# flydog-sdr/FlyDog_SDR_GPS

Hardware: AMD Instinct MI355X
Metric: IQ Msamples/s ingested (waterfall + GPS acq); value = GPS acq, BASELINE configs[1] (higher is better)
Workload: dtype f32

## Files before the change

### flydog_sdr_gps_amd/csrc/kg_acq.hip

```cpp
#include "kg_common.h"
#include "kg_fft.h"
#include "kg_acq_tables.h"

#include <math.h>
#include <stdlib.h>
#include <vector>

#define SUB      4096
#define NTAPS    31
#define DECIM    4


enum { SRC_BITS = 0, SRC_IQ16 = 1, SRC_CHIPS = 2 };

__constant__ float c_hb_even[16] = {
    -0.010233f,  0.010668f, -0.016324f,  0.024377f, -0.036482f,  0.056990f, -0.101993f,
     0.316926f,  0.316926f, -0.101993f,  0.056990f, -0.036482f,  0.024377f, -0.016324f,
     0.010668f, -0.010233f,
};
#define HB_CENTRE 0.500009f

KG_DEV float bipolar(int bit) { return bit ? -1.0f : 1.0f; }

template <int SRC>
KG_DEV cf acq_source(const void *__restrict__ src, int i, int nvalid, int nchips, int boc)
{
    if (i >= nvalid) return cf{0.f, 0.f};
    if constexpr (SRC == SRC_BITS) {
        const uint8_t *p = (const uint8_t *) src;
        const int bit = (p[i >> 3] >> (i & 7)) & 1;
        const int ph = i & 3;
        const int ls = ph < 2, lc = (ph == 0) | (ph == 3);
        return cf{bipolar(bit ^ ls), bipolar(bit ^ lc)};
    } else if constexpr (SRC == SRC_IQ16) {
        const short2 v = ((const short2 *) src)[i];
        const float a = (float) v.x, b = (float) v.y;
        switch (i & 3) {
        case 0:  return cf{a, b};
        case 1:  return cf{b, -a};
        case 2:  return cf{-a, -b};
        default: return cf{-b, a};
        }
    } else {
        const uint8_t *p = (const uint8_t *) src;
        const int chip = p[(i >> 4) % nchips];
        const int b11 = boc ? ((i & 15) >= 8) : 0;
        return cf{bipolar(chip ^ b11), 0.f};
    }
}

KG_DEV cf hb_tap(const float2 *x)
{
    cf acc = kg_scale(kg_ld(&x[0]), c_hb_even[0]);
#pragma unroll
    for (int j = 1; j < 16; j++) acc = acc + kg_scale(kg_ld(&x[2 * j]), c_hb_even[j]);
    acc = acc + kg_scale(kg_ld(&x[(NTAPS - 1) / 2]), HB_CENTRE);
    return acc;
}

#define FE_TILE 256
#define FE_NY1  (2 * FE_TILE + NTAPS - 2)
#define FE_NX   (2 * FE_NY1 + NTAPS - 2)

template <int SRC>
__global__ __launch_bounds__(256) void acq_frontend_kernel(const uint8_t *__restrict__ src,
                                                          size_t src_stride, int nvalid, int nchips, int boc,
                                                          float2 *__restrict__ td, int fft_len)
{
    __shared__ float2 xs[FE_NX + 1];
    __shared__ float2 y1[FE_NY1 + 1];
    const int tid = threadIdx.x;
    const int o0 = blockIdx.x * FE_TILE;
    const void *s = src + (size_t) blockIdx.y * src_stride;
    for (int u = tid; u < FE_NX; u += 256) kg_st(&xs[u], acq_source<SRC>(s, 4 * o0 + u, nvalid, nchips, boc));
    __syncthreads();
    for (int u = tid; u < FE_NY1; u += 256) kg_st(&y1[u], hb_tap(&xs[2 * u]));
    __syncthreads();
    kg_st(&td[(size_t) blockIdx.y * fft_len + o0 + tid], hb_tap(&y1[2 * tid]));
}

#define STAMP(i)                                                                      \
    do {                                                                              \
        if (STAMPS) {                                                                 \
            __builtin_amdgcn_sched_barrier(0);                                        \
            if (threadIdx.x == 0 && blockIdx.x == 0 && blockIdx.y == 0)               \
                stamps[i] = __builtin_amdgcn_s_memrealtime();                         \
            __builtin_amdgcn_sched_barrier(0);                                        \
        }                                                                             \
    } while (0)

template <bool STAMPS>
__global__ __launch_bounds__(256) void acq_fft_sub_kernel(const float2 *__restrict__ td,
                                                         float2 *__restrict__ scratch,
                                                         const float2 *__restrict__ tab4096, int P,
                                                         unsigned long long *__restrict__ stamps)
{
    extern __shared__ __attribute__((aligned(16))) float2 smem[];
    const int t = threadIdx.x, g = blockIdx.x;
    const float2 *in = td + (size_t) blockIdx.y * P * SUB;
    float2 *out = scratch + ((size_t) blockIdx.y * P + g) * SUB;
    STAMP(0);
    cf x[16], y[16];
#pragma unroll
    for (int j = 0; j < 16; j++) x[j] = kg_ld(&in[P * (t + 256 * j) + g]);
    kg_tw4096 tw;
    kg_tw4096_load(tw, tab4096, t);
    if (STAMPS) { asm volatile("s_waitcnt vmcnt(0)" ::: "memory"); }
    STAMP(1);
    kg_subfft4096<-1>(x, y, smem, smem + SUB, tw, t);
    STAMP(2);
#pragma unroll
    for (int m = 0; m < 16; m++) kg_st(&out[t + 256 * m], y[m]);
    if (STAMPS) { asm volatile("s_waitcnt vmcnt(0)" ::: "memory"); }
    STAMP(3);
}

template <int P>
__global__ __launch_bounds__(256) void acq_fft_combine_kernel(const float2 *__restrict__ scratch,
                                                             float2 *__restrict__ planes,
                                                             float2 *__restrict__ planes_b,
                                                             size_t planes_stride,
                                                             const float2 *__restrict__ tabN,
                                                             int halo)
{
    static_assert(P == 4 || P == 16, "N = 16384 or 65536");
    const int k = blockIdx.x * 256 + threadIdx.x;
    const float2 *f = scratch + (size_t) blockIdx.y * (P * SUB);
    cf v[P];
    v[0] = kg_ld(&f[k]);
#pragma unroll
    for (int g = 1; g < P; g++) v[g] = kg_cmulc(kg_ld(&f[g * SUB + k]), kg_ld(&tabN[g * k]));
    cf fq[P];
    if constexpr (P == 4) {
        kg_radix4<-1>(v[0], v[1], v[2], v[3]);
#pragma unroll
        for (int q = 0; q < 4; q++) fq[q] = v[q];
    } else {
        kg_radix16<-1>(v, fq);
    }
    if (planes) {
        const int row = 2 * (256 + 2 * halo), plane = 8 * row;
        float2 *o = planes + (size_t) blockIdx.y * planes_stride + (size_t) (k & (P - 1)) * plane;
#pragma unroll
        for (int q = 0; q < P; q++) {
            const int k1 = k / P + (SUB / P) * q;
            const int tt = k1 & 255, j = k1 >> 8;
            kg_st(&o[(j >> 1) * row + 2 * (tt + halo) + (j & 1)], fq[q]);
            if (tt < halo) {
                const int jj = (j - 1) & 15;
                kg_st(&o[(jj >> 1) * row + 2 * (tt + 256 + halo) + (jj & 1)], fq[q]);
            }
            if (tt >= 256 - halo) {
                const int jj = (j + 1) & 15;
                kg_st(&o[(jj >> 1) * row + 2 * (tt - 256 + halo) + (jj & 1)], fq[q]);
            }
        }
    }
    if (planes_b) {
        const int row = 2 * (512 + 2 * halo), plane = 4 * row;
        float2 *o = planes_b + (size_t) blockIdx.y * planes_stride + (size_t) (k & (P - 1)) * plane;
#pragma unroll
        for (int q = 0; q < P; q++) {
            const int k1 = k / P + (SUB / P) * q;
            const int ii = k1 & 511, j = k1 >> 9;
            kg_st(&o[(j >> 1) * row + 2 * (ii + halo) + (j & 1)], fq[q]);
            if (ii < halo) {
                const int jj = (j - 1) & 7;
                kg_st(&o[(jj >> 1) * row + 2 * (ii + 512 + halo) + (jj & 1)], fq[q]);
            }
            if (ii >= 512 - halo) {
                const int jj = (j + 1) & 7;
                kg_st(&o[(jj >> 1) * row + 2 * (ii - 512 + halo) + (jj & 1)], fq[q]);
            }
        }
    }
}

struct acq_red { float p; int i; float s; int pad; };

#define ACQ_CLAIM_STRIDE 32
#define ACQ_LDS_BYTES (2 * SUB * sizeof(float2) + 16)

struct __attribute__((aligned(16))) acq_part { float p; int i; float s; int pad; };

struct acq_pair_desc {
    int data_off;
    int code_off;
    int limit;
    int out;
};

struct acq_cell_desc { int data_off, code_off, dop, limit, out; };

struct acq_walk {
    int npairs;
    int ndop, dop_lo;
};

template <int P, bool STAMPS = false>
__global__ __launch_bounds__(256, 2) void acq_correlate_kernel(
    const float2 *__restrict__ data,
    const float2 *__restrict__ code,
    const float2 *__restrict__ tab4096, const float2 *__restrict__ tabN,
    const float2 *__restrict__ comb,
    const acq_pair_desc *__restrict__ pairs,
    int *__restrict__ claim,
    acq_walk walk,
    int halo,
// ... 585 lines not shown
            cells[(size_t) pd.out + di] = c;
        } else {
            c = cells[(size_t) pd.out + di];
        }
        if (c.snr > bs) { bs = c.snr; bd = di; bidx = c.idx; }
    }
#pragma unroll
    for (int off = 32; off >= 1; off >>= 1) {
        const float os = __shfl_xor(bs, off);
        const int od = __shfl_xor(bd, off), oi = __shfl_xor(bidx, off);
        if (os > bs || (os == bs && od < bd)) { bs = os; bd = od; bidx = oi; }
    }
    if (lane == 0) {
        kg_acq_result r;
        r.valid = bs > 0.f ? 1 : 0;
        r.snr = r.valid ? bs : 0.f;
        r.dop = r.valid ? dop_lo + bd : 0;
        r.idx = r.valid ? bidx : 0;
        out[p] = r;
    }
}

struct kg_acq {
    kg_ctx *ctx;
    int max_sats, dop_lo, dop_hi, ndop, max_blocks;
    int nsamples;
    int fft_len;
    int P;
    size_t in_stride;
    int halo;
    size_t code_len;
    const float2 *d_tabN;
    kg_dbuf<float2> own_tabN;
    kg_dbuf<float2> d_comb;
    kg_dbuf<float2> d_quart;
    kg_dbuf<float2> d_comb8;
    int grid8;
    kg_dbuf<float2> d_code;
    kg_dbuf<float2> d_data;
    kg_dbuf<float2> d_data_b;
    std::vector<char> code_layout;
    kg_dbuf<float2> d_td;
    kg_dbuf<float2> d_td_code;
    kg_dbuf<float2> d_fsub;
    kg_dbuf<float2> d_fsub_code;
    kg_dbuf<uint8_t> d_in;
    kg_hbuf<uint8_t> h_pin[4];
    hipEvent_t ev_pin[4];
    int pin_next;
    kg_hbuf<uint8_t> h_batch; size_t batch_cap; hipEvent_t ev_batch;
    hipStream_t cstream; hipEvent_t ev_in_free; bool in_free_set;
    kg_dbuf<uint8_t> d_chips;
    kg_dbuf<kg_acq_cell> d_cells;
    kg_dbuf<acq_part> d_parts;
    kg_dbuf<kg_acq_result> d_results;
    kg_dbuf<int> d_claim;
    std::vector<int> limits, code_set;
    std::vector<int> last_sats;
    const acq_pair_desc *d_pairs1, *d_pairs4;
    unsigned long pairs_seq;
    int last_first, last_nblocks, last_nsats, np1, np4, table_nblocks;
    hipStream_t fstream;
    bool own_fstream;
    std::vector<hipEvent_t> ev_ready, ev_done;
    std::vector<int> ready_of, done_of;
    int grid1;
};

static inline __host__ __device__ size_t plane_pos(int k1, int halo_col, int H, int layout)
{
    if (layout == 0) {
        const int t = k1 & 255, j = k1 >> 8, row = 2 * (256 + 2 * H);
        return (size_t) (j >> 1) * row + 2 * (t + halo_col + H) + (j & 1);
    }
    const int t = k1 & 511, j = k1 >> 9, row = 2 * (512 + 2 * H);
    return (size_t) (j >> 1) * row + 2 * (t + halo_col + H) + (j & 1);
}
static inline size_t spec_len(int P, int H) { return (size_t) P * 8 * 2 * (256 + 2 * H); }
// ... 11 lines not shown

static void to_planes(const float *nat, std::vector<float2> &pl, int P, int H, int layout)
{
    const size_t plane = plane_len(H, layout);
    const int T = layout == 0 ? 256 : 512, J = SUB / T;
    pl.assign(spec_len(P, H), make_float2(0.f, 0.f));
    for (int k = 0; k < P * SUB; k++) {
        const float2 v = make_float2(nat[2 * k], nat[2 * k + 1]);
        const int k1 = k / P, t = k1 & (T - 1), j = k1 / T;
        float2 *p = pl.data() + (size_t) (k % P) * plane;
        p[plane_pos(k1, 0, H, layout)] = v;
        if (t < H) p[plane_pos(t + T * ((j - 1) & (J - 1)), T, H, layout)] = v;
        if (t >= T - H) p[plane_pos(t + T * ((j + 1) & (J - 1)), -T, H, layout)] = v;
    }
}
static void from_planes(const std::vector<float2> &pl, float *nat, int P, int H, int layout)
{
    const size_t plane = plane_len(H, layout);
    for (int k = 0; k < P * SUB; k++) {
        const float2 v = pl[(size_t) (k % P) * plane + plane_pos(k / P, 0, H, layout)];
        nat[2 * k] = v.x; nat[2 * k + 1] = v.y;
    }
}

static float2 unit_root(long k, long n)
{
    float2 r;
    kg_unit_root_f(k, n, &r.x, &r.y);
    return r;
}

template <int SRC>
static int launch_frontend(kg_acq *a, hipStream_t st, const uint8_t *d_src, size_t stride, int nbatch,
                           int nvalid, int nchips, int boc, float2 *d_td, float2 *d_scratch,
                           float2 *d_planes, float2 *d_planes_b, size_t planes_stride, int halo)
{
    kg_ctx *c = a->ctx;
    hipLaunchKernelGGL(acq_frontend_kernel<SRC>, dim3(a->fft_len / FE_TILE, nbatch), dim3(256), 0,
                       st, d_src, stride, nvalid, nchips, boc, d_td, a->fft_len);
    KG_HIP(hipGetLastError());
    hipLaunchKernelGGL(acq_fft_sub_kernel<false>, dim3(a->P, nbatch), dim3(256), 2 * SUB * sizeof(float2),
                       st, (const float2 *) d_td, d_scratch, (const float2 *) c->d_tab4096, a->P,
                       (unsigned long long *) nullptr);
    KG_HIP(hipGetLastError());
    if (a->P == 4)
        hipLaunchKernelGGL(acq_fft_combine_kernel<4>, dim3(SUB / 256, nbatch), dim3(256), 0, st,
                           (const float2 *) d_scratch, d_planes, d_planes_b, planes_stride,
                           (const float2 *) a->d_tabN, halo);
    else
        hipLaunchKernelGGL(acq_fft_combine_kernel<16>, dim3(SUB / 256, nbatch), dim3(256), 0, st,
                           (const float2 *) d_scratch, d_planes, d_planes_b, planes_stride,
                           (const float2 *) a->d_tabN, halo);
    KG_HIP(hipGetLastError());
    return KG_OK;
}

static int acq_init(kg_acq *a)
{
    kg_ctx *ctx = a->ctx;
    const int max_sats = a->max_sats, max_blocks = a->max_blocks, N = a->fft_len, P = a->P;
    {
        const int m = (a->dop_hi > -a->dop_lo ? a->dop_hi : -a->dop_lo);
        a->halo = (m + P - 1) / P + 2;
        a->code_len = spec_len(P, a->halo);
    }
    a->limits.assign(max_sats, 0); a->code_set.assign(max_sats, 0); a->code_layout.assign(max_sats, 0);
    a->last_first = a->last_nblocks = a->last_nsats = a->np1 = a->np4 = a->table_nblocks = 0;
    a->d_pairs1 = a->d_pairs4 = nullptr; a->pairs_seq = 0;
    a->in_stride = (size_t) a->nsamples * 4;
    const size_t spec = sizeof(float2) * N;
    if (N == 16384) a->d_tabN = ctx->d_tab16384;
    else {
        std::vector<float2> h(N);
        for (int k = 0; k < N; k++) h[k] = unit_root(k, N);
        KG_TRY(a->own_tabN.alloc(N, "kg_acq_create: twiddle table"));
        a->d_tabN = a->own_tabN;
        KG_HIP(hipMemcpy(a->own_tabN, h.data(), spec, hipMemcpyHostToDevice));
    }
    {
        std::vector<float2> comb(P * KG_ACQ_ROWK + (P == 16 ? 4 * 256 : 0)), quart(P * 4);
        static_assert(sizeof(float2) == 2 * sizeof(float), "float2 = (re, im)");
        kg_acq_row_consts(P, &comb[0].x);
        if (P == 16) kg_acq_mid_factors(N, &comb[P * KG_ACQ_ROWK].x);
        for (int k2 = 0; k2 < P; k2++)
            for (int q = 0; q < 4; q++) quart[4 * k2 + q] = unit_root((long) q * k2, P);
        KG_TRY(a->d_comb.alloc(comb.size(), "kg_acq_create: row constants"));
        KG_TRY(a->d_quart.alloc(quart.size(), "kg_acq_create: quarter factors"));
        KG_HIP(hipMemcpy(a->d_comb, comb.data(), sizeof(float2) * comb.size(), hipMemcpyHostToDevice));
        KG_HIP(hipMemcpy(a->d_quart, quart.data(), sizeof(float2) * quart.size(), hipMemcpyHostToDevice));
        std::vector<float2> comb8(P * 4);
        for (int k2 = 0; k2 < P; k2++)
            for (int k = 0; k < 4; k++) comb8[4 * k2 + k] = unit_root((long) (k + 1) * k2, N / 512);
        KG_TRY(a->d_comb8.alloc(comb8.size(), "kg_acq_create: combine constants"));
        KG_HIP(hipMemcpy(a->d_comb8, comb8.data(), sizeof(float2) * comb8.size(), hipMemcpyHostToDevice));
    }
    KG_TRY(a->d_code.alloc(a->code_len * max_sats, "kg_acq_create: code spectra"));
    KG_TRY(a->d_data.alloc((size_t) N * max_blocks, "kg_acq_create: data spectra"));
    KG_TRY(a->d_td.alloc((size_t) N * max_blocks, "kg_acq_create: decimated samples"));
    KG_TRY(a->d_td_code.alloc(N, "kg_acq_create: decimated samples"));
    KG_TRY(a->d_fsub.alloc((size_t) N * max_blocks, "kg_acq_create: sub-transforms"));
    KG_TRY(a->d_fsub_code.alloc(N, "kg_acq_create: sub-transforms"));
    KG_TRY(a->d_in.alloc(a->in_stride * max_blocks, "kg_acq_create: input staging"));
    for (int k = 0; k < 4; k++) {
        KG_TRY(a->h_pin[k].alloc(a->in_stride, "kg_acq_create: pinned input slots"));
        KG_HIP(hipEventCreateWithFlags(&a->ev_pin[k], hipEventDisableTiming));
    }
    KG_HIP(hipEventCreateWithFlags(&a->ev_batch, hipEventDisableTiming));
    KG_HIP(hipEventCreateWithFlags(&a->ev_in_free, hipEventDisableTiming));
    KG_TRY(kg_stream_get(ctx->device, &a->cstream));
    KG_TRY(a->d_chips.alloc(8192, "kg_acq_create: chips"));
    KG_TRY(a->d_cells.alloc((size_t) max_blocks * max_sats * a->ndop, "kg_acq_create: cells"));
    KG_TRY(a->d_parts.alloc(4 * (size_t) max_blocks * max_sats * a->ndop, "kg_acq_create: wave records"));
    KG_TRY(a->d_results.alloc((size_t) max_blocks * max_sats, "kg_acq_create: results"));
    KG_TRY(a->d_claim.alloc(16 * ACQ_CLAIM_STRIDE, "kg_acq_create: claim counters"));
    KG_HIP(hipMemset(a->d_claim, 0, sizeof(int) * 16 * ACQ_CLAIM_STRIDE));
    {
        const char *e = kg_tuning_env("KIWIGPU_ACQ_FRONT_STREAM");
        if (e && e[0] == '1') {
            KG_TRY(kg_stream_get(ctx->device, &a->fstream));
            a->own_fstream = true;
        }
    }
    a->ready_of.assign(max_blocks, -1); a->done_of.assign(max_blocks, -1);
    a->ev_ready.reserve(max_blocks); a->ev_done.reserve(max_blocks);
    for (int b = 0; b < max_blocks; b++) {
        hipEvent_t e1, e2;
        KG_HIP(hipEventCreateWithFlags(&e1, hipEventDisableTiming));
        a->ev_ready.push_back(e1);
        KG_HIP(hipEventCreateWithFlags(&e2, hipEventDisableTiming));
        a->ev_done.push_back(e2);
    }
    KG_HIP(hipMemset(a->d_data, 0, spec * max_blocks));
    KG_HIP(hipFuncSetAttribute((const void *) acq_fft_sub_kernel<false>,
                               hipFuncAttributeMaxDynamicSharedMemorySize, 2 * SUB * sizeof(float2)));
    KG_HIP(hipFuncSetAttribute((const void *) acq_fft_sub_kernel<true>,
                               hipFuncAttributeMaxDynamicSharedMemorySize, 2 * SUB * sizeof(float2)));
    int occ1 = 0;
#define ACQ_SETUP(PP)                                                                                          \
    KG_HIP(hipFuncSetAttribute((const void *) acq_correlate_kernel<PP>,                                       \
                               hipFuncAttributeMaxDynamicSharedMemorySize, ACQ_LDS_BYTES));                   \
    KG_HIP(hipOccupancyMaxActiveBlocksPerMultiprocessor(&occ1, acq_correlate_kernel<PP>, 256,                 \
                                                        ACQ_LDS_BYTES));
    if (P == 4) { ACQ_SETUP(4) } else { ACQ_SETUP(16) }
#undef ACQ_SETUP
    if (occ1 < 1) occ1 = 1;
    if (const char *e = kg_tuning_env("KIWIGPU_ACQ_WGS_PER_CU")) {
        const int v = atoi(e);
        if (v >= 1 && v < occ1) occ1 = v;
    }
    a->grid1 = (ctx->num_cus * occ1) & ~7;
    if (P == 4)
        KG_HIP(hipFuncSetAttribute((const void *) acq_correlate8_kernel<4>,
                                   hipFuncAttributeMaxDynamicSharedMemorySize, ACQ8_LDS_BYTES));
    else
        KG_HIP(hipFuncSetAttribute((const void *) acq_correlate8_kernel<16>,
                                   hipFuncAttributeMaxDynamicSharedMemorySize, ACQ8_LDS_BYTES));
    a->grid8 = ctx->num_cus & ~7;
    if (a->grid8 < 8) a->grid8 = 8;
    if (a->grid1 < 8) a->grid1 = 8;
    return KG_OK;
}

extern "C" {

int kg_acq_create_shape(kg_ctx *ctx, int max_sats, int dop_lo, int dop_hi, int max_blocks, int nsamples,
                        int fft_len, kg_acq **out)
{
    int rc = kg_ctx_use(ctx);
    if (rc) return rc;
// ... 84 lines not shown
    }
    a->limits[sat] = limit;
    a->code_layout[sat] = layout;
    a->code_set[sat] = 1;
    a->last_sats.clear();
    return KG_OK;
}

static int acq_patch_overrun(kg_acq *a, int sat)
{
    if (sat < 0 || sat >= a->max_sats || !a->code_set[sat]) return KG_OK;
    const bool have_next = sat + 1 < a->max_sats && a->code_set[sat + 1];
    const int n = a->P * a->halo;
    hipLaunchKernelGGL(acq_code_overrun_kernel, dim3((n + 63) / 64), dim3(64), 0, a->ctx->stream,
                       a->d_code + (size_t) sat * a->code_len, a->code_layout[sat],
                       have_next ? (const float2 *) (a->d_code + (size_t) (sat + 1) * a->code_len) : (const float2 *) nullptr,
                       have_next ? a->code_layout[sat + 1] : 0, a->P, a->halo);
    KG_HIP(hipGetLastError());
    return KG_OK;
}

int kg_acq_set_code(kg_acq *a, int sat, const uint8_t *chips, int nchips, int boc, int limit)
{
    KG_REQUIRE(a && chips, KG_ERR_INVALID, "kg_acq_set_code: null argument");
    int rc = kg_ctx_use(a->ctx);
    if (rc) return rc;
    KG_REQUIRE(nchips >= 1 && nchips <= 8192, KG_ERR_INVALID, "kg_acq_set_code: nchips %d", nchips);
    for (int i = 0; i < nchips; i++)
        KG_REQUIRE(chips[i] <= 1, KG_ERR_INVALID, "kg_acq_set_code: chips[%d] = %d is not 0/1", i, chips[i]);
    KG_TRY(set_limit(a, sat, limit));
    KG_HIP(hipMemcpyAsync(a->d_chips, chips, nchips, hipMemcpyHostToDevice, a->ctx->stream));
    float2 *d_sv = a->d_code + (size_t) sat * a->code_len;
    rc = launch_frontend<SRC_CHIPS>(a, a->ctx->stream, a->d_chips, 0, 1, DECIM * a->fft_len, nchips, boc ? 1 : 0,
                                    a->d_td_code, a->d_fsub_code, a->code_layout[sat] ? nullptr : d_sv,
                                    a->code_layout[sat] ? d_sv : nullptr, a->code_len, a->halo);
    if (rc) return rc;
    if ((rc = acq_patch_overrun(a, sat)) || (rc = acq_patch_overrun(a, sat - 1))) return rc;
    KG_HIP(hipStreamSynchronize(a->ctx->stream));
    return KG_OK;
}

int kg_acq_set_code_fft(kg_acq *a, int sat, const float *code_fft, int limit)
{
    KG_REQUIRE(a && code_fft, KG_ERR_INVALID, "kg_acq_set_code_fft: null argument");
    int rc = kg_ctx_use(a->ctx);
    if (rc) return rc;
    KG_TRY(set_limit(a, sat, limit));
    std::vector<float2> pl;
    to_planes(code_fft, pl, a->P, a->halo, a->code_layout[sat]);
    KG_HIP(hipMemcpyAsync(a->d_code + (size_t) sat * a->code_len, pl.data(), sizeof(float2) * a->code_len,
                          hipMemcpyHostToDevice, a->ctx->stream));
    if ((rc = acq_patch_overrun(a, sat)) || (rc = acq_patch_overrun(a, sat - 1))) return rc;
    KG_HIP(hipStreamSynchronize(a->ctx->stream));
    return KG_OK;
}

static int get_planes(kg_acq *a, const float2 *d, float *nat, int H, int layout)
{
    std::vector<float2> pl(spec_len(a->P, H));
    KG_HIP(hipStreamSynchronize(a->fstream));
    KG_HIP(hipMemcpyAsync(pl.data(), d, sizeof(float2) * pl.size(), hipMemcpyDeviceToHost, a->ctx->stream));
    KG_HIP(hipStreamSynchronize(a->ctx->stream));
    from_planes(pl, nat, a->P, H, layout);
    return KG_OK;
}

int kg_acq_get_code_fft(kg_acq *a, int sat, float *code_fft)
// ... 47 lines not shown
static int wait_once(hipStream_t st, const std::vector<hipEvent_t> &ev, const std::vector<int> &of, int b, int n)
{
    for (int i = b; i < b + n; i++) {
        const int e = of[i];
        if (e < 0) continue;
        bool seen = false;
        for (int k = b; k < i && !seen; k++) seen = of[k] == e;
        if (!seen) KG_HIP(hipStreamWaitEvent(st, ev[e], 0));
    }
    return KG_OK;
}
static int front_begin(kg_acq *a, int b, int n = 1)
{
    if (!a->own_fstream) return KG_OK;
    return wait_once(a->fstream, a->ev_done, a->done_of, b, n);
}
static int front_end(kg_acq *a, int b, int n = 1)
{
    if (!a->own_fstream) return KG_OK;
    KG_HIP(hipEventRecord(a->ev_ready[b], a->fstream));
    for (int i = b; i < b + n; i++) a->ready_of[i] = b;
    return KG_OK;
}

}

template <int SRC>
static int sample_dev(kg_acq *a, int first, int nblocks, const void *d_src, size_t stride)
{
    int rc;
    KG_TRY(front_begin(a, first, nblocks));
    const size_t off = (size_t) first * a->fft_len;
    rc = launch_frontend<SRC>(a, a->fstream, (const uint8_t *) d_src, stride, nblocks, a->nsamples, 0, 0,
                              a->d_td + off, a->d_fsub + off, a->d_data + off, a->d_data_b ? a->d_data_b + off : nullptr,
                              a->fft_len, 0);
    if (rc) return rc;
    return front_end(a, first, nblocks);
}

extern "C" {

int kg_acq_sample_bits_dev(kg_acq *a, int block, const void *d_packed)
{
    int rc = check_block(a, block, d_packed, "kg_acq_sample_bits_dev");
    if (rc) return rc;
    return sample_dev<SRC_BITS>(a, block, 1, d_packed, 0);
}

int kg_acq_sample_bits(kg_acq *a, int block, const uint8_t *packed)
{
    int rc = check_block(a, block, packed, "kg_acq_sample_bits");
    if (rc) return rc;
    uint8_t *stage = a->d_in + a->in_stride * block;
    if ((rc = stage_host_block(a, stage, packed, (size_t) a->nsamples / 8))) return rc;
    KG_TRY(sample_dev<SRC_BITS>(a, block, 1, stage, 0));
    return staging_consumed(a);
}

int kg_acq_sample_iq16_dev(kg_acq *a, int block, const void *d_iq)
{
    int rc = check_block(a, block, d_iq, "kg_acq_sample_iq16_dev");
    if (rc) return rc;
    KG_REQUIRE(((uintptr_t) d_iq & 3) == 0, KG_ERR_INVALID, "kg_acq_sample_iq16_dev: pointer not 4-byte aligned");
    return sample_dev<SRC_IQ16>(a, block, 1, d_iq, 0);
}

int kg_acq_sample_iq16_batch_dev(kg_acq *a, int first, int nblocks, const void *d_iq, size_t stride_bytes)
// ... 242 lines not shown
        return KG_OK;
    }
    KG_REQUIRE(a->np1 > 0, KG_ERR_STATE, "kg_acq_debug_corr_stamps: no C/A SV in the list");
    unsigned long long *d = nullptr;
    const size_t bytes = sizeof(unsigned long long) * (512 + 4 * 1024);
    KG_REQUIRE(a->grid1 <= 1024, KG_ERR_STATE, "kg_acq_debug_corr_stamps: grid %d", a->grid1);
    kg_scope tmp(a->ctx);
    KG_TRY(tmp.alloc(&d, 512 + 4 * 1024, "kg_acq_debug_corr_stamps"));
    KG_HIP(hipMemset(d, 0, bytes));
    KG_HIP(hipMemsetAsync(a->d_claim, 0, sizeof(int) * 16 * ACQ_CLAIM_STRIDE, st));
    if (a->P == 4) {
        KG_HIP(hipFuncSetAttribute((const void *) acq_correlate_kernel<4, true>,
                                   hipFuncAttributeMaxDynamicSharedMemorySize, ACQ_LDS_BYTES));
        launch_correlate<4, true>(a, st, 0, a->d_pairs1, a->np1, d);
    } else {
        KG_HIP(hipFuncSetAttribute((const void *) acq_correlate_kernel<16, true>,
                                   hipFuncAttributeMaxDynamicSharedMemorySize, ACQ_LDS_BYTES));
        launch_correlate<16, true>(a, st, 0, a->d_pairs1, a->np1, d);
    }
    KG_HIP(hipGetLastError());
    KG_HIP(hipMemsetAsync(a->d_claim, 0, sizeof(int) * 16 * ACQ_CLAIM_STRIDE, st));
    KG_HIP(hipStreamSynchronize(st));
    KG_HIP(hipMemcpy(stamps, d, bytes, hipMemcpyDeviceToHost));
    return KG_OK;
}

int kg_acq_debug_fft_stamps(kg_acq *a, int block, unsigned long long *stamps, int n)
{
    int rc = check_block(a, block, stamps, "kg_acq_debug_fft_stamps");
    if (rc) return rc;
    KG_REQUIRE(n >= 4, KG_ERR_INVALID, "kg_acq_debug_fft_stamps: need room for 4 stamps");
    kg_ctx *c = a->ctx;
    unsigned long long *d = nullptr;
    kg_scope tmp(c);
    KG_TRY(tmp.alloc(&d, 8, "kg_acq_debug_fft_stamps"));
    KG_HIP(hipStreamSynchronize(a->fstream));
    for (int rep = 0; rep < 3; rep++) {
        hipLaunchKernelGGL(acq_fft_sub_kernel<true>, dim3(a->P, 1), dim3(256), 2 * SUB * sizeof(float2),
                           c->stream, (const float2 *) (a->d_td + (size_t) block * a->fft_len),
                           a->d_fsub + (size_t) block * a->fft_len, (const float2 *) c->d_tab4096, a->P, d);
        KG_HIP(hipGetLastError());
        KG_HIP(hipStreamSynchronize(c->stream));
    }
    KG_HIP(hipMemcpy(stamps, d, 4 * sizeof(unsigned long long), hipMemcpyDeviceToHost));
    return KG_OK;
}

}
```

### flydog_sdr_gps_amd/csrc/kg_fft.h

```cpp
#pragma once

#include <hip/hip_runtime.h>
#include "kg_tables.h"

typedef float cf __attribute__((ext_vector_type(2)));

#define KG_DEV __device__ __forceinline__

KG_DEV cf kg_scale(cf a, float s) { return a * cf{s, s}; }
KG_DEV cf kg_ld(const float2 *p) { return *reinterpret_cast<const cf *>(p); }
KG_DEV void kg_st(float2 *p, cf v) { *reinterpret_cast<cf *>(p) = v; }
KG_DEV cf kg_ld_tile(const float2 *p) { return *(const volatile cf __attribute__((address_space(3))) *) p; }
KG_DEV void kg_st_tile(float2 *p, cf v) { *(volatile cf __attribute__((address_space(3))) *) p = v; }

KG_DEV cf kg_cmul(cf a, cf w)
{
    cf r, d;
    asm("v_pk_mul_f32 %0, %1, %2 op_sel_hi:[1,0]" : "=v"(r) : "v"(a), "v"(w));
    asm("v_pk_fma_f32 %0, %1, %2, %3 op_sel:[1,1,0] op_sel_hi:[0,1,1] neg_lo:[0,1,0]"
        : "=v"(d) : "v"(a), "v"(w), "v"(r));
    return d;
}
KG_DEV cf kg_cmulc(cf a, cf w)
{
// ... 322 lines not shown
        kg_addsub_sj<SIGN>(x[4 + b], x[12 + b], d02[b], d13[b]);
    }
}

#define kg_pin() __builtin_amdgcn_sched_barrier(0)
template <int SIGN, class H> KG_DEV void kg_tw_radix16_h(cf (&x)[16], cf (&y)[16], const kg_tw15 &w, H hook)
{
    kg_radix16_stage1_tw<SIGN>(x, w, hook);
    kg_radix16_stage2f<SIGN>(x, y, hook);
}
template <int SIGN, class H> KG_DEV void kg_tw_radix16_hk(cf (&x)[16], cf (&y)[16], const kg_tw15 &w, const cf (&k)[12], H hook)
{
    kg_radix16_stage1_tw<SIGN>(x, w, hook);
    kg_radix16_stage2f_k<SIGN>(x, y, k, hook);
}
template <int SIGN, class H> KG_DEV void kg_cc_radix16_h(const cf (&c)[16], const cf (&d)[16], cf (&y)[16], H hook)
{
    cf x[16];
    kg_radix16_stage1_cc<SIGN>(c, d, x, hook);
    kg_radix16_stage2f<SIGN>(x, y, hook);
}

struct kg_tw4096 { kg_tw15 p1, p2; };

KG_DEV void kg_tw4096_load(kg_tw4096 &tw, const float2 *__restrict__ tab4096, int t)
{
#pragma unroll
    for (int j = 1; j < 16; j++) {
        tw.p1.w[j - 1] = kg_ld(&tab4096[(j * (t & 15)) << 4]);
        tw.p2.w[j - 1] = kg_ld(&tab4096[j * t]);
    }
}

template <int SIGN> KG_DEV void kg_twiddle16(cf (&x)[16], const kg_tw15 &w)
{
    kg_cmul4v<(SIGN < 0)>(x[1], x[2], x[3], x[4], w.w[0], w.w[1], w.w[2], w.w[3]);
    kg_cmul4v<(SIGN < 0)>(x[5], x[6], x[7], x[8], w.w[4], w.w[5], w.w[6], w.w[7]);
    kg_cmul4v<(SIGN < 0)>(x[9], x[10], x[11], x[12], w.w[8], w.w[9], w.w[10], w.w[11]);
    kg_cmul3v<(SIGN < 0)>(x[13], x[14], x[15], w.w[12], w.w[13], w.w[14]);
}

#define KG_STAMP(on, ptr, i)                                                          \
    do {                                                                              \
        if (on) {                                                                     \
            __builtin_amdgcn_sched_barrier(0);                                        \
            if ((ptr) != nullptr) (ptr)[i] = __builtin_amdgcn_s_memtime();            \
            __builtin_amdgcn_sched_barrier(0);                                        \
        }                                                                             \
    } while (0)

template <int SIGN, bool STAMPS = false>
KG_DEV void kg_subfft4096_a(cf (&x)[16], cf (&y)[16], float2 *tileA, float2 *tileB,
                            const kg_tw4096 &tw, int t, unsigned long long *st = nullptr)
{
    const int tl = t & 15, th = t >> 4;
    const int rd = t ^ (th & 15);
    kg_radix16<SIGN>(x, y);
    KG_STAMP(STAMPS, st, 0);
#pragma unroll
    for (int m = 0; m < 16; m++) kg_st_tile(&tileA[16 * t + (m ^ tl)], y[m]);
    KG_STAMP(STAMPS, st, 1);
    __syncthreads();
    KG_STAMP(STAMPS, st, 2);
#pragma unroll
    for (int j = 0; j < 16; j++) x[j] = kg_ld_tile(&tileA[rd + 256 * j]);
    if (STAMPS) asm volatile("s_waitcnt lgkmcnt(0)" ::: "memory");
// ... 225 lines not shown
```

Baseline: 2771.

## Fuse sub-FFT and combine into one decimation-in-frequency planes kernel

Replaces the two-pass FFT (strided 4096-point sub-FFTs written to scratch, then a radix-4/16 combine kernel that scatters into planes) with one kernel. Each block first applies the radix-P butterfly and twiddle to coalesced inputs (decimation in frequency), then runs a 4096-point sub-FFT and writes plane rows directly with vector stores. This removes the scratch round trip, one launch and strided loads. The front-end kernel also reads source samples four at a time with vector loads into split even/odd shared buffers, and sub-FFT twiddles are precomputed into coalesced per-thread rows. The cost is more arithmetic per load and more register pressure in the fused kernel.

After: 2778, median of 6. No clear change (+0.3%).

```diff
diff --git a/flydog_sdr_gps_amd/csrc/kg_acq.hip b/flydog_sdr_gps_amd/csrc/kg_acq.hip
--- a/flydog_sdr_gps_amd/csrc/kg_acq.hip
+++ b/flydog_sdr_gps_amd/csrc/kg_acq.hip
@@ -22,61 +22,102 @@
 
 KG_DEV float bipolar(int bit) { return bit ? -1.0f : 1.0f; }
 
+KG_DEV void acq_st2(float2 *p, cf a, cf b)
+{
+    typedef float cf4 __attribute__((ext_vector_type(4)));
+    *reinterpret_cast<cf4 *>(p) = __builtin_shufflevector(a, b, 0, 1, 2, 3);
+}
+
 template <int SRC>
-KG_DEV cf acq_source(const void *__restrict__ src, int i, int nvalid, int nchips, int boc)
-{
-    if (i >= nvalid) return cf{0.f, 0.f};
+KG_DEV void acq_source4(const void *__restrict__ src, int i0, int nvalid, int nchips, int boc, bool src16, cf (&v)[4])
+{
+    const cf zero = cf{0.f, 0.f};
     if constexpr (SRC == SRC_BITS) {
         const uint8_t *p = (const uint8_t *) src;
-        const int bit = (p[i >> 3] >> (i & 7)) & 1;
-        const int ph = i & 3;
-        const int ls = ph < 2, lc = (ph == 0) | (ph == 3);
-        return cf{bipolar(bit ^ ls), bipolar(bit ^ lc)};
+        const int nib = i0 < nvalid ? p[i0 >> 3] >> (i0 & 7) : 0;
+#pragma unroll
+        for (int k = 0; k < 4; k++) {
+            const int bit = (nib >> k) & 1;
+            const int ls = k < 2, lc = (k == 0) | (k == 3);
+            v[k] = i0 + k < nvalid ? cf{bipolar(bit ^ ls), bipolar(bit ^ lc)} : zero;
+        }
     } else if constexpr (SRC == SRC_IQ16) {
-        const short2 v = ((const short2 *) src)[i];
-        const float a = (float) v.x, b = (float) v.y;
-        switch (i & 3) {
-        case 0:  return cf{a, b};
-        case 1:  return cf{b, -a};
-        case 2:  return cf{-a, -b};
-        default: return cf{-b, a};
-        }
+        const int *p = (const int *) src + i0;
+        int w[4] = {0, 0, 0, 0};
+        if (i0 + 3 < nvalid) {
+            if (src16) {
+                const int4 q = *(const int4 *) p;
+                w[0] = q.x; w[1] = q.y; w[2] = q.z; w[3] = q.w;
+            } else {
+#pragma unroll
+                for (int k = 0; k < 4; k++) w[k] = p[k];
+            }
+        } else {
+#pragma unroll
+            for (int k = 0; k < 4; k++)
+                if (i0 + k < nvalid) w[k] = p[k];
+        }
+        float a[4], b[4];
+#pragma unroll
+        for (int k = 0; k < 4; k++) { a[k] = (float) (short) (w[k] & 0xffff); b[k] = (float) (short) (w[k] >> 16); }
+        v[0] = i0 < nvalid ? cf{a[0], b[0]} : zero;
+        v[1] = i0 + 1 < nvalid ? cf{b[1], -a[1]} : zero;
+        v[2] = i0 + 2 < nvalid ? cf{-a[2], -b[2]} : zero;
+        v[3] = i0 + 3 < nvalid ? cf{-b[3], a[3]} : zero;
     } else {
         const uint8_t *p = (const uint8_t *) src;
-        const int chip = p[(i >> 4) % nchips];
-        const int b11 = boc ? ((i & 15) >= 8) : 0;
-        return cf{bipolar(chip ^ b11), 0.f};
-    }
-}
-
-KG_DEV cf hb_tap(const float2 *x)
-{
-    cf acc = kg_scale(kg_ld(&x[0]), c_hb_even[0]);
-#pragma unroll
-    for (int j = 1; j < 16; j++) acc = acc + kg_scale(kg_ld(&x[2 * j]), c_hb_even[j]);
-    acc = acc + kg_scale(kg_ld(&x[(NTAPS - 1) / 2]), HB_CENTRE);
+        const int chip = i0 < nvalid ? p[(i0 >> 4) % nchips] : 0;
+        const int b11 = boc ? ((i0 & 15) >= 8) : 0;
+        const float c = bipolar(chip ^ b11);
+#pragma unroll
+        for (int k = 0; k < 4; k++) v[k] = i0 + k < nvalid ? cf{c, 0.f} : zero;
+    }
+}
+
+KG_DEV cf hb_tap(const float2 *e, const float2 *o)
+{
+    cf acc = kg_scale(kg_ld(&e[0]), c_hb_even[0]);
+#pragma unroll
+    for (int j = 1; j < 16; j++) acc = acc + kg_scale(kg_ld(&e[j]), c_hb_even[j]);
+    acc = acc + kg_scale(kg_ld(o), HB_CENTRE);
     return acc;
 }
 
 #define FE_TILE 256
+#define FE_THREADS 320
 #define FE_NY1  (2 * FE_TILE + NTAPS - 2)
 #define FE_NX   (2 * FE_NY1 + NTAPS - 2)
+#define FE_NQ   ((FE_NX + 3) / 4)
+#define FE_NYH  (FE_TILE + 16)
 
 template <int SRC>
-__global__ __launch_bounds__(256) void acq_frontend_kernel(const uint8_t *__restrict__ src,
-                                                          size_t src_stride, int nvalid, int nchips, int boc,
-                                                          float2 *__restrict__ td, int fft_len)
-{
-    __shared__ float2 xs[FE_NX + 1];
-    __shared__ float2 y1[FE_NY1 + 1];
+__global__ __launch_bounds__(FE_THREADS) void acq_frontend_kernel(const uint8_t *__restrict__ src,
+                                                                 size_t src_stride, int nvalid, int nchips, int boc,
+                                                                 float2 *__restrict__ td, int fft_len)
+{
+    __shared__ __attribute__((aligned(16))) float2 xe[2 * FE_NQ];
+    __shared__ __attribute__((aligned(16))) float2 xo[2 * FE_NQ];
+    __shared__ float2 y1[2 * FE_NYH];
+    float2 *ye = y1, *yo = y1 + FE_NYH;
     const int tid = threadIdx.x;
     const int o0 = blockIdx.x * FE_TILE;
-    const void *s = src + (size_t) blockIdx.y * src_stride;
-    for (int u = tid; u < FE_NX; u += 256) kg_st(&xs[u], acq_source<SRC>(s, 4 * o0 + u, nvalid, nchips, boc));
+    const uint8_t *s = src + (size_t) blockIdx.y * src_stride;
+    constexpr int QT = (FE_NQ + FE_THREADS - 1) / FE_THREADS;
+    cf v[QT][4];
+#pragma unroll
+    for (int k = 0; k < QT; k++)
+        if (tid + k * FE_THREADS < FE_NQ)
+            acq_source4<SRC>(s, 4 * (o0 + tid + k * FE_THREADS), nvalid, nchips, boc, ((uintptr_t) s & 15) == 0, v[k]);
+#pragma unroll
+    for (int k = 0; k < QT; k++)
+        if (tid + k * FE_THREADS < FE_NQ) {
+            acq_st2(&xe[2 * (tid + k * FE_THREADS)], v[k][0], v[k][2]);
+            acq_st2(&xo[2 * (tid + k * FE_THREADS)], v[k][1], v[k][3]);
+        }
     __syncthreads();
-    for (int u = tid; u < FE_NY1; u += 256) kg_st(&y1[u], hb_tap(&xs[2 * u]));
+    for (int u = tid; u < FE_NY1; u += FE_THREADS) kg_st(&((u & 1) ? yo : ye)[u >> 1], hb_tap(&xe[u], &xo[u + 7]));
     __syncthreads();
-    kg_st(&td[(size_t) blockIdx.y * fft_len + o0 + tid], hb_tap(&y1[2 * tid]));
+    for (int u = tid; u < FE_TILE; u += FE_THREADS) kg_st(&td[(size_t) blockIdx.y * fft_len + o0 + u], hb_tap(&ye[u], &yo[u + 7]));
 }
 
 #define STAMP(i)                                                                      \
@@ -89,91 +130,124 @@
         }                                                                             \
     } while (0)
 
-template <bool STAMPS>
-__global__ __launch_bounds__(256) void acq_fft_sub_kernel(const float2 *__restrict__ td,
-                                                         float2 *__restrict__ scratch,
-                                                         const float2 *__restrict__ tab4096, int P,
-                                                         unsigned long long *__restrict__ stamps)
-{
+__constant__ float2 c_w16[16] = {
+    {KG_W16[0][0], KG_W16[0][1]},   {KG_W16[1][0], KG_W16[1][1]},   {KG_W16[2][0], KG_W16[2][1]},   {KG_W16[3][0], KG_W16[3][1]},
+    {KG_W16[4][0], KG_W16[4][1]},   {KG_W16[5][0], KG_W16[5][1]},   {KG_W16[6][0], KG_W16[6][1]},   {KG_W16[7][0], KG_W16[7][1]},
+    {KG_W16[8][0], KG_W16[8][1]},   {KG_W16[9][0], KG_W16[9][1]},   {KG_W16[10][0], KG_W16[10][1]}, {KG_W16[11][0], KG_W16[11][1]},
+    {KG_W16[12][0], KG_W16[12][1]}, {KG_W16[13][0], KG_W16[13][1]}, {KG_W16[14][0], KG_W16[14][1]}, {KG_W16[15][0], KG_W16[15][1]},
+};
+
+template <int RR> KG_DEV cf acq_radix4_one(cf x0, cf x1, cf x2, cf x3)
+{
+    if constexpr (RR == 0) return (x0 + x2) + (x1 + x3);
+    else if constexpr (RR == 2) return (x0 + x2) - (x1 + x3);
+    else if constexpr (RR == 1) return kg_subj(x0 - x2, x1 - x3);
+    else return kg_addj(x0 - x2, x1 - x3);
+}
+
+template <int P, int RR> KG_DEV void acq_planes_load(cf (&x)[16], const float2 *__restrict__ in,
+                                                     const float2 *__restrict__ tabN, int t, int r)
+{
+#pragma unroll
+    for (int j = 0; j < 16; j++) {
+        const float2 *p = in + t + 256 * j;
+        if constexpr (P == 4) {
+            x[j] = acq_radix4_one<RR>(kg_ld(p), kg_ld(p + SUB), kg_ld(p + 2 * SUB), kg_ld(p + 3 * SUB));
+        } else {
+            cf s[4];
+#pragma unroll
+            for (int b = 0; b < 4; b++)
+                s[b] = acq_radix4_one<RR>(kg_ld(p + b * SUB), kg_ld(p + (4 + b) * SUB), kg_ld(p + (8 + b) * SUB),
+                                          kg_ld(p + (12 + b) * SUB));
+            cf u1, u2, u3;
+            if (r == 0) { u1 = s[1]; u2 = s[2]; u3 = s[3]; }
+            else {
+                u1 = kg_cmulc(s[1], kg_ld(&c_w16[r]));
+                u2 = kg_cmulc(s[2], kg_ld(&c_w16[(2 * r) & 15]));
+                u3 = kg_cmulc(s[3], kg_ld(&c_w16[(3 * r) & 15]));
+            }
+            x[j] = (s[0] + u2) + (u1 + u3);
+        }
+    }
+    if (r != 0) {
+#pragma unroll
+        for (int j = 0; j < 16; j++) x[j] = kg_cmulc(x[j], kg_ld(&tabN[(t + 256 * j) * r]));
+    }
+}
+
+template <int P, bool STAMPS>
+__global__ __launch_bounds__(256) void acq_fft_planes_kernel(const float2 *__restrict__ td,
+                                                            float2 *__restrict__ planes,
+                                                            float2 *__restrict__ planes_b,
+                                                            size_t planes_stride,
+                                                            const float2 *__restrict__ tw_rows,
+                                                            const float2 *__restrict__ tabN,
+                                                            int halo,
+                                                            unsigned long long *__restrict__ stamps)
+{
+    static_assert(P == 4 || P == 16, "N = 16384 or 65536");
     extern __shared__ __attribute__((aligned(16))) float2 smem[];
-    const int t = threadIdx.x, g = blockIdx.x;
-    const float2 *in = td + (size_t) blockIdx.y * P * SUB;
-    float2 *out = scratch + ((size_t) blockIdx.y * P + g) * SUB;
+    const int t = threadIdx.x, r = blockIdx.x;
+    const float2 *in = td + (size_t) blockIdx.y * (P * SUB);
     STAMP(0);
     cf x[16], y[16];
-#pragma unroll
-    for (int j = 0; j < 16; j++) x[j] = kg_ld(&in[P * (t + 256 * j) + g]);
+    switch (r & 3) {
+    case 0:  acq_planes_load<P, 0>(x, in, tabN, t, r); break;
+    case 1:  acq_planes_load<P, 1>(x, in, tabN, t, r); break;
+    case 2:  acq_planes_load<P, 2>(x, in, tabN, t, r); break;
+    default: acq_planes_load<P, 3>(x, in, tabN, t, r); break;
+    }
     kg_tw4096 tw;
-    kg_tw4096_load(tw, tab4096, t);
+    kg_tw4096_load_rows(tw, tw_rows, t);
     if (STAMPS) { asm volatile("s_waitcnt vmcnt(0)" ::: "memory"); }
     STAMP(1);
     kg_subfft4096<-1>(x, y, smem, smem + SUB, tw, t);
     STAMP(2);
-#pragma unroll
-    for (int m = 0; m < 16; m++) kg_st(&out[t + 256 * m], y[m]);
+    if (planes) {
+        const int row = 2 * (256 + 2 * halo), plane = 8 * row;
+        float2 *o = planes + (size_t) blockIdx.y * planes_stride + (size_t) r * plane;
+#pragma unroll
+        for (int i = 0; i < 8; i++) acq_st2(&o[i * row + 2 * (t + halo)], y[2 * i], y[2 * i + 1]);
+        if (t < halo) {
+#pragma unroll
+            for (int j = 0; j < 16; j++) {
+                const int jj = (j - 1) & 15;
+                kg_st(&o[(jj >> 1) * row + 2 * (t + 256 + halo) + (jj & 1)], y[j]);
+            }
+        }
+        if (t >= 256 - halo) {
+#pragma unroll
+            for (int j = 0; j < 16; j++) {
+                const int jj = (j + 1) & 15;
+                kg_st(&o[(jj >> 1) * row + 2 * (t - 256 + halo) + (jj & 1)], y[j]);
+            }
+        }
+    }
+    if (planes_b) {
+        const int row = 2 * (512 + 2 * halo), plane = 4 * row;
+        float2 *o = planes_b + (size_t) blockIdx.y * planes_stride + (size_t) r * plane;
+#pragma unroll
+        for (int i = 0; i < 4; i++) {
+            acq_st2(&o[i * row + 2 * (t + halo)], y[4 * i], y[4 * i + 2]);
+            acq_st2(&o[i * row + 2 * (t + 256 + halo)], y[4 * i + 1], y[4 * i + 3]);
+        }
+        if (t < halo) {
+#pragma unroll
+            for (int j = 0; j < 8; j++) {
+                const int jj = (j - 1) & 7;
+                kg_st(&o[(jj >> 1) * row + 2 * (t + 512 + halo) + (jj & 1)], y[2 * j]);
+            }
+        }
+        if (t >= 256 - halo) {
+#pragma unroll
+            for (int j = 0; j < 8; j++) {
+                const int jj = (j + 1) & 7;
+                kg_st(&o[(jj >> 1) * row + 2 * (t - 256 + halo) + (jj & 1)], y[2 * j + 1]);
+            }
+        }
+    }
     if (STAMPS) { asm volatile("s_waitcnt vmcnt(0)" ::: "memory"); }
     STAMP(3);
-}
-
-template <int P>
-__global__ __launch_bounds__(256) void acq_fft_combine_kernel(const float2 *__restrict__ scratch,
-                                                             float2 *__restrict__ planes,
-                                                             float2 *__restrict__ planes_b,
-                                                             size_t planes_stride,
-                                                             const float2 *__restrict__ tabN,
-                                                             int halo)
-{
-    static_assert(P == 4 || P == 16, "N = 16384 or 65536");
-    const int k = blockIdx.x * 256 + threadIdx.x;
-    const float2 *f = scratch + (size_t) blockIdx.y * (P * SUB);
-    cf v[P];
-    v[0] = kg_ld(&f[k]);
-#pragma unroll
-    for (int g = 1; g < P; g++) v[g] = kg_cmulc(kg_ld(&f[g * SUB + k]), kg_ld(&tabN[g * k]));
-    cf fq[P];
-    if constexpr (P == 4) {
-        kg_radix4<-1>(v[0], v[1], v[2], v[3]);
-#pragma unroll
-        for (int q = 0; q < 4; q++) fq[q] = v[q];
-    } else {
-        kg_radix16<-1>(v, fq);
-    }
-    if (planes) {
-        const int row = 2 * (256 + 2 * halo), plane = 8 * row;
-        float2 *o = planes + (size_t) blockIdx.y * planes_stride + (size_t) (k & (P - 1)) * plane;
-#pragma unroll
-        for (int q = 0; q < P; q++) {
-            const int k1 = k / P + (SUB / P) * q;
-            const int tt = k1 & 255, j = k1 >> 8;
-            kg_st(&o[(j >> 1) * row + 2 * (tt + halo) + (j & 1)], fq[q]);
-            if (tt < halo) {
-                const int jj = (j - 1) & 15;
-                kg_st(&o[(jj >> 1) * row + 2 * (tt + 256 + halo) + (jj & 1)], fq[q]);
-            }
-            if (tt >= 256 - halo) {
-                const int jj = (j + 1) & 15;
-                kg_st(&o[(jj >> 1) * row + 2 * (tt - 256 + halo) + (jj & 1)], fq[q]);
-            }
-        }
-    }
-    if (planes_b) {
-        const int row = 2 * (512 + 2 * halo), plane = 4 * row;
-        float2 *o = planes_b + (size_t) blockIdx.y * planes_stride + (size_t) (k & (P - 1)) * plane;
-#pragma unroll
-        for (int q = 0; q < P; q++) {
-            const int k1 = k / P + (SUB / P) * q;
-            const int ii = k1 & 511, j = k1 >> 9;
-            kg_st(&o[(j >> 1) * row + 2 * (ii + halo) + (j & 1)], fq[q]);
-            if (ii < halo) {
-                const int jj = (j - 1) & 7;
-                kg_st(&o[(jj >> 1) * row + 2 * (ii + 512 + halo) + (jj & 1)], fq[q]);
-            }
-            if (ii >= 512 - halo) {
-                const int jj = (j + 1) & 7;
-                kg_st(&o[(jj >> 1) * row + 2 * (ii - 512 + halo) + (jj & 1)], fq[q]);
-            }
-        }
-    }
 }
 
 struct acq_red { float p; int i; float s; int pad; };
@@ -825,6 +899,7 @@
     size_t code_len;
     const float2 *d_tabN;
     kg_dbuf<float2> own_tabN;
+    kg_dbuf<float2> d_tw_rows;
     kg_dbuf<float2> d_comb;
     kg_dbuf<float2> d_quart;
     kg_dbuf<float2> d_comb8;
@@ -835,8 +910,6 @@
     std::vector<char> code_layout;
     kg_dbuf<float2> d_td;
     kg_dbuf<float2> d_td_code;
-    kg_dbuf<float2> d_fsub;
-    kg_dbuf<float2> d_fsub_code;
     kg_dbuf<uint8_t> d_in;
     kg_hbuf<uint8_t> h_pin[4];
     hipEvent_t ev_pin[4];
@@ -914,25 +987,20 @@
 
 template <int SRC>
 static int launch_frontend(kg_acq *a, hipStream_t st, const uint8_t *d_src, size_t stride, int nbatch,
-                           int nvalid, int nchips, int boc, float2 *d_td, float2 *d_scratch,
+                           int nvalid, int nchips, int boc, float2 *d_td,
                            float2 *d_planes, float2 *d_planes_b, size_t planes_stride, int halo)
 {
-    kg_ctx *c = a->ctx;
-    hipLaunchKernelGGL(acq_frontend_kernel<SRC>, dim3(a->fft_len / FE_TILE, nbatch), dim3(256), 0,
+    hipLaunchKernelGGL(acq_frontend_kernel<SRC>, dim3(a->fft_len / FE_TILE, nbatch), dim3(FE_THREADS), 0,
                        st, d_src, stride, nvalid, nchips, boc, d_td, a->fft_len);
     KG_HIP(hipGetLastError());
-    hipLaunchKernelGGL(acq_fft_sub_kernel<false>, dim3(a->P, nbatch), dim3(256), 2 * SUB * sizeof(float2),
-                       st, (const float2 *) d_td, d_scratch, (const float2 *) c->d_tab4096, a->P,
-                       (unsigned long long *) nullptr);
-    KG_HIP(hipGetLastError());
     if (a->P == 4)
-        hipLaunchKernelGGL(acq_fft_combine_kernel<4>, dim3(SUB / 256, nbatch), dim3(256), 0, st,
-                           (const float2 *) d_scratch, d_planes, d_planes_b, planes_stride,
-                           (const float2 *) a->d_tabN, halo);
+        hipLaunchKernelGGL((acq_fft_planes_kernel<4, false>), dim3(4, nbatch), dim3(256), 2 * SUB * sizeof(float2), st,
+                           (const float2 *) d_td, d_planes, d_planes_b, planes_stride, (const float2 *) a->d_tw_rows,
+                           (const float2 *) a->d_tabN, halo, (unsigned long long *) nullptr);
     else
-        hipLaunchKernelGGL(acq_fft_combine_kernel<16>, dim3(SUB / 256, nbatch), dim3(256), 0, st,
-                           (const float2 *) d_scratch, d_planes, d_planes_b, planes_stride,
-                           (const float2 *) a->d_tabN, halo);
+        hipLaunchKernelGGL((acq_fft_planes_kernel<16, false>), dim3(16, nbatch), dim3(256), 2 * SUB * sizeof(float2), st,
+                           (const float2 *) d_td, d_planes, d_planes_b, planes_stride, (const float2 *) a->d_tw_rows,
+                           (const float2 *) a->d_tabN, halo, (unsigned long long *) nullptr);
     KG_HIP(hipGetLastError());
     return KG_OK;
 }
@@ -958,6 +1026,13 @@
         KG_TRY(a->own_tabN.alloc(N, "kg_acq_create: twiddle table"));
         a->d_tabN = a->own_tabN;
         KG_HIP(hipMemcpy(a->own_tabN, h.data(), spec, hipMemcpyHostToDevice));
+    }
+    {
+        std::vector<float2> tab(SUB), rows(KG_TW4096_ROWS);
+        KG_HIP(hipMemcpy(tab.data(), ctx->d_tab4096, sizeof(float2) * SUB, hipMemcpyDeviceToHost));
+        kg_tw4096_rows(tab.data(), rows.data());
+        KG_TRY(a->d_tw_rows.alloc(rows.size(), "kg_acq_create: twiddle rows"));
+        KG_HIP(hipMemcpy(a->d_tw_rows, rows.data(), sizeof(float2) * rows.size(), hipMemcpyHostToDevice));
     }
     {
         std::vector<float2> comb(P * KG_ACQ_ROWK + (P == 16 ? 4 * 256 : 0)), quart(P * 4);
@@ -980,8 +1055,6 @@
     KG_TRY(a->d_data.alloc((size_t) N * max_blocks, "kg_acq_create: data spectra"));
     KG_TRY(a->d_td.alloc((size_t) N * max_blocks, "kg_acq_create: decimated samples"));
     KG_TRY(a->d_td_code.alloc(N, "kg_acq_create: decimated samples"));
-    KG_TRY(a->d_fsub.alloc((size_t) N * max_blocks, "kg_acq_create: sub-transforms"));
-    KG_TRY(a->d_fsub_code.alloc(N, "kg_acq_create: sub-transforms"));
     KG_TRY(a->d_in.alloc(a->in_stride * max_blocks, "kg_acq_create: input staging"));
     for (int k = 0; k < 4; k++) {
         KG_TRY(a->h_pin[k].alloc(a->in_stride, "kg_acq_create: pinned input slots"));
@@ -1013,10 +1086,17 @@
         a->ev_done.push_back(e2);
     }
     KG_HIP(hipMemset(a->d_data, 0, spec * max_blocks));
-    KG_HIP(hipFuncSetAttribute((const void *) acq_fft_sub_kernel<false>,
-                               hipFuncAttributeMaxDynamicSharedMemorySize, 2 * SUB * sizeof(float2)));
-    KG_HIP(hipFuncSetAttribute((const void *) acq_fft_sub_kernel<true>,
-                               hipFuncAttributeMaxDynamicSharedMemorySize, 2 * SUB * sizeof(float2)));
+    if (P == 4) {
+        KG_HIP(hipFuncSetAttribute((const void *) acq_fft_planes_kernel<4, false>,
+                                   hipFuncAttributeMaxDynamicSharedMemorySize, 2 * SUB * sizeof(float2)));
+        KG_HIP(hipFuncSetAttribute((const void *) acq_fft_planes_kernel<4, true>,
+                                   hipFuncAttributeMaxDynamicSharedMemorySize, 2 * SUB * sizeof(float2)));
+    } else {
+        KG_HIP(hipFuncSetAttribute((const void *) acq_fft_planes_kernel<16, false>,
+                                   hipFuncAttributeMaxDynamicSharedMemorySize, 2 * SUB * sizeof(float2)));
+        KG_HIP(hipFuncSetAttribute((const void *) acq_fft_planes_kernel<16, true>,
+                                   hipFuncAttributeMaxDynamicSharedMemorySize, 2 * SUB * sizeof(float2)));
+    }
     int occ1 = 0;
 #define ACQ_SETUP(PP)                                                                                          \
     KG_HIP(hipFuncSetAttribute((const void *) acq_correlate_kernel<PP>,                                       \
@@ -1167,7 +1247,7 @@
     KG_HIP(hipMemcpyAsync(a->d_chips, chips, nchips, hipMemcpyHostToDevice, a->ctx->stream));
     float2 *d_sv = a->d_code + (size_t) sat * a->code_len;
     rc = launch_frontend<SRC_CHIPS>(a, a->ctx->stream, a->d_chips, 0, 1, DECIM * a->fft_len, nchips, boc ? 1 : 0,
-                                    a->d_td_code, a->d_fsub_code, a->code_layout[sat] ? nullptr : d_sv,
+                                    a->d_td_code, a->code_layout[sat] ? nullptr : d_sv,
                                     a->code_layout[sat] ? d_sv : nullptr, a->code_len, a->halo);
     if (rc) return rc;
     if ((rc = acq_patch_overrun(a, sat)) || (rc = acq_patch_overrun(a, sat - 1))) return rc;
@@ -1281,7 +1361,7 @@
     KG_TRY(front_begin(a, first, nblocks));
     const size_t off = (size_t) first * a->fft_len;
     rc = launch_frontend<SRC>(a, a->fstream, (const uint8_t *) d_src, stride, nblocks, a->nsamples, 0, 0,
-                              a->d_td + off, a->d_fsub + off, a->d_data + off, a->d_data_b ? a->d_data_b + off : nullptr,
+                              a->d_td + off, a->d_data + off, a->d_data_b ? a->d_data_b + off : nullptr,
                               a->fft_len, 0);
     if (rc) return rc;
     return front_end(a, first, nblocks);
@@ -1590,13 +1670,21 @@
     KG_REQUIRE(n >= 4, KG_ERR_INVALID, "kg_acq_debug_fft_stamps: need room for 4 stamps");
     kg_ctx *c = a->ctx;
     unsigned long long *d = nullptr;
+    float2 *d_out = nullptr;
     kg_scope tmp(c);
     KG_TRY(tmp.alloc(&d, 8, "kg_acq_debug_fft_stamps"));
+    KG_TRY(tmp.alloc(&d_out, a->fft_len, "kg_acq_debug_fft_stamps"));
     KG_HIP(hipStreamSynchronize(a->fstream));
+    const float2 *d_in = a->d_td + (size_t) block * a->fft_len;
     for (int rep = 0; rep < 3; rep++) {
-        hipLaunchKernelGGL(acq_fft_sub_kernel<true>, dim3(a->P, 1), dim3(256), 2 * SUB * sizeof(float2),
-                           c->stream, (const float2 *) (a->d_td + (size_t) block * a->fft_len),
-                           a->d_fsub + (size_t) block * a->fft_len, (const float2 *) c->d_tab4096, a->P, d);
+        if (a->P == 4)
+            hipLaunchKernelGGL((acq_fft_planes_kernel<4, true>), dim3(4, 1), dim3(256), 2 * SUB * sizeof(float2), c->stream,
+                               d_in, d_out, (float2 *) nullptr, (size_t) 0, (const float2 *) a->d_tw_rows,
+                               (const float2 *) a->d_tabN, 0, d);
+        else
+            hipLaunchKernelGGL((acq_fft_planes_kernel<16, true>), dim3(16, 1), dim3(256), 2 * SUB * sizeof(float2), c->stream,
+                               d_in, d_out, (float2 *) nullptr, (size_t) 0, (const float2 *) a->d_tw_rows,
+                               (const float2 *) a->d_tabN, 0, d);
         KG_HIP(hipGetLastError());
         KG_HIP(hipStreamSynchronize(c->stream));
     }
diff --git a/flydog_sdr_gps_amd/csrc/kg_fft.h b/flydog_sdr_gps_amd/csrc/kg_fft.h
--- a/flydog_sdr_gps_amd/csrc/kg_fft.h
+++ b/flydog_sdr_gps_amd/csrc/kg_fft.h
@@ -378,6 +378,24 @@
     }
 }
 
+KG_DEV void kg_tw4096_load_rows(kg_tw4096 &tw, const float2 *__restrict__ tabT, int t)
+{
+#pragma unroll
+    for (int j = 1; j < 16; j++) {
+        tw.p1.w[j - 1] = kg_ld(&tabT[(j - 1) * 256 + t]);
+        tw.p2.w[j - 1] = kg_ld(&tabT[(15 + j - 1) * 256 + t]);
+    }
+}
+#define KG_TW4096_ROWS (30 * 256)
+static inline void kg_tw4096_rows(const float2 *tab4096, float2 *tabT)
+{
+    for (int j = 1; j < 16; j++)
+        for (int t = 0; t < 256; t++) {
+            tabT[(j - 1) * 256 + t] = tab4096[(j * (t & 15)) << 4];
+            tabT[(15 + j - 1) * 256 + t] = tab4096[j * t];
+        }
+}
+
 template <int SIGN> KG_DEV void kg_twiddle16(cf (&x)[16], const kg_tw15 &w)
 {
     kg_cmul4v<(SIGN < 0)>(x[1], x[2], x[3], x[4], w.w[0], w.w[1], w.w[2], w.w[3]);
```
